# nsp5488/go_raytracer

Hardware: AMD Instinct MI355X
Metric: Msamples/sec (pixels×spp/s) + wall-clock, Cornell Box 800×800×1024spp (higher is better)
Workload: dtype f32

## Files before the change

### go_raytracer_amd/__init__.py

```python
import ctypes as C
import weakref

import numpy as np

from . import _lib
from ._lib import (RT_FT_ALL, RT_FT_BOX, RT_NOISE_MARBLE, RT_NOISE_PERLIN,
                   RT_NOISE_TURBULENT, RtAccumInfo, RtAov, RtCamera, RtDenoiseOpts,
                   RtDenoiseVarOpts, RtCameraDerived, RtError, RtRenderOpts, RtSceneInfo, RtStats, RtTreeView,
                   check, lib)

__all__ = ["Tree", "Camera", "Scene", "Accumulator", "quantize", "format_ppm", "device_count", "RtError",
           "tune", "untune", "tuning", "tune_knobs", "tune_from_env",
           "demo_scene", "DEMO_SCENES", "LoadObjOptions", "DefaultLoadOptions", "quantize_device",
           "format_ppm_device", "denoise", "denoise_device", "denoise_var", "denoise_var_device",
           "RtDenoiseVarOpts"]

DEMO_SCENES = ("book1", "book2", "book3", "simple_light", "quads", "cornell", "cornell_smoke",
               "model")


def _d3(v):
    return _lib.D3(*[float(x) for x in v])


# ... 377 lines not shown
        check(lib().rt_scene_export_qbvh(self._p, None, C.byref(ni), None, C.byref(nn), C.byref(root)))
        items = np.zeros((max(ni.value, 0), 16), np.uint32)
        nodes = np.zeros((max(nn.value, 0), 32), np.uint32)
        check(lib().rt_scene_export_qbvh(self._p, items.ctypes.data or None, C.byref(ni),
                                         nodes.ctypes.data or None, C.byref(nn), C.byref(root)))
        return items, nodes, int(root.value)

    def export_records(self, fill=True):
        ns, sn, nb, counts = C.c_int32(), C.c_int32(), C.c_int32(), (C.c_int32 * 7)()
        check(lib().rt_scene_export_records(self._p, None, C.byref(ns), counts, C.byref(sn), C.byref(nb)))
        pairs = np.zeros((4 * ns.value + sn.value, 4), np.uint32)
        if fill:
            check(lib().rt_scene_export_records(self._p, pairs.ctypes.data or None, C.byref(ns), counts,
                                                C.byref(sn), C.byref(nb)))
        return pairs, ns.value, tuple(counts), sn.value, nb.value

    MODES = {"auto": 0, "wavefront": 1, "fused": 2}

    @staticmethod
    def _opts(seed, device, rank, nranks, path_slots, chunk, profile, stream, mode="auto"):
        o = RtRenderOpts()
        o.mode = Scene.MODES[mode]
        o.seed = seed
        o.device = device
        o.rank = rank
        o.nranks = nranks
        o.path_slots = path_slots
        o.chunk = chunk
        o.flags = _lib.RT_FLAG_PROFILE if profile else 0
        o.stream = stream
# ... 411 lines not shown
```

### go_raytracer_amd/_lib.py

```python
import ctypes as C
import os

_HERE = os.path.dirname(os.path.abspath(__file__))
LIB_PATH = os.environ.get("RT_AMD_LIB") or os.path.join(_HERE, "librt_amd.so")

RT_OK = 0
RT_ERR_INVALID = -1
RT_ERR_UNSUPPORTED = -2
RT_ERR_DEVICE = -3
RT_ERR_OOM = -4
RT_ERR_IO = -5

RT_TEX_SOLID, RT_TEX_CHECKER, RT_TEX_IMAGE, RT_TEX_NOISE = range(4)
RT_NOISE_PERLIN, RT_NOISE_MARBLE, RT_NOISE_TURBULENT = 1, 2, 3
(RT_MAT_LAMBERTIAN, RT_MAT_METAL, RT_MAT_DIELECTRIC, RT_MAT_DIFFUSE_LIGHT,
 RT_MAT_ISOTROPIC) = range(5)
(RT_NODE_LIST, RT_NODE_BVH, RT_NODE_SPHERE, RT_NODE_QUAD, RT_NODE_TRIANGLE,
 RT_NODE_TRANSLATE, RT_NODE_ROTATE_Y, RT_NODE_MEDIUM) = range(8)
RT_FLAG_PROFILE = 1
RT_FLAG_GATHER_RCCL = 2
RT_FT_SPHERE, RT_FT_TRI, RT_FT_METAL, RT_FT_DIEL = 1, 2, 4, 8
RT_FT_MEDIA, RT_FT_CHECKER, RT_FT_IMAGE, RT_FT_NOISE = 16, 32, 64, 128
RT_FT_BOX = 256
RT_FT_ALL = 511
# ... 167 lines not shown
                                C.POINTER(RtObjInfo)]),
    "rt_tree_get_view": (_I, [_P, C.POINTER(RtTreeView)]),
    "rt_camera_derive": (_I, [C.POINTER(RtCamera), C.POINTER(RtCameraDerived)]),
    "rt_scene_create": (_I, [_P, _I, _I, C.POINTER(_P)]),
    "rt_scene_destroy": (_I, [_P]),
    "rt_scene_info_get": (_I, [_P, C.POINTER(RtSceneInfo)]),
    "rt_scene_export_bvh": (_I, [_P, C.c_void_p, C.POINTER(C.c_int32), C.c_void_p,
                                 C.POINTER(C.c_int32), C.POINTER(C.c_uint32)]),
    "rt_scene_export_bvh8": (_I, [_P, C.c_void_p, C.POINTER(C.c_int32), C.c_void_p,
                                  C.POINTER(C.c_int32)]),
    "rt_scene_export_qbvh": (_I, [_P, C.c_void_p, C.POINTER(C.c_int32), C.c_void_p,
                                  C.POINTER(C.c_int32), C.POINTER(C.c_uint32)]),
    "rt_scene_export_records": (_I, [_P, C.c_void_p, C.POINTER(C.c_int32), C.POINTER(C.c_int32),
                                     C.POINTER(C.c_int32), C.POINTER(C.c_int32)]),
    "rt_scene_export_prim_bounds": (_I, [_P, C.c_void_p, C.POINTER(C.c_int32)]),
    "rt_render": (_I, [_P, C.POINTER(RtCamera), C.POINTER(RtRenderOpts), C.c_void_p,
                       C.POINTER(RtStats)]),
    "rt_render_device": (_I, [_P, C.POINTER(RtCamera), C.POINTER(RtRenderOpts), C.c_void_p,
                              C.POINTER(RtStats)]),
    "rt_render_multi": (_I, [_P, C.POINTER(RtCamera), C.POINTER(RtRenderOpts),
                             C.POINTER(C.c_int32), C.c_int32, C.c_void_p, C.POINTER(RtStats)]),
    "rt_render_multi_device": (_I, [_P, C.POINTER(RtCamera), C.POINTER(RtRenderOpts),
                                    C.POINTER(C.c_int32), C.c_int32, C.c_void_p,
                                    C.POINTER(RtStats)]),
    "rt_quantize": (_I, [C.c_void_p, C.c_int64, C.c_void_p]),
    "rt_format_ppm": (C.c_int64, [C.c_void_p, _I, _I, C.c_void_p, C.c_int64]),
    "rt_progress": (_I, [_P, C.POINTER(C.c_uint64), C.POINTER(C.c_uint64)]),
    "rt_quantize_device": (_I, [C.c_void_p, C.c_int64, C.c_void_p, _I, C.c_void_p]),
    "rt_format_ppm_device": (C.c_int64, [C.c_void_p, _I, _I, C.c_void_p, C.c_int64, _I,
                                         C.c_void_p]),
# ... 59 lines not shown
```

### go_raytracer_amd/csrc/host_records.cpp

```cpp
#include <math.h>
#include <string.h>

#include <algorithm>

#include "rt_internal.h"

namespace rt {

void build_leaf_records(const HostScene& h, std::vector<F4>& recs) {
  recs.assign(4 * h.refs.size(), F4{0, 0, 0, 0});
  for (size_t i = 0; i < h.refs.size(); ++i) make_record(h, h.refs[i], &recs[4 * i]);
}
void build_light_records(const HostScene& h, std::vector<F4>& recs) {
  recs.assign(8 * std::max<size_t>(h.lights.size(), 1), F4{0, 0, 0, 0});
  for (size_t i = 0; i < h.lights.size(); ++i) {
    const uint32_t ref = h.lights[i].ref;
    if (ref == PRIM_NONE || (ref >> 30) != PRIM_QUAD) continue;
    make_record(h, ref, &recs[8 * i]);
    const F4* q = &h.quad[5 * (size_t)(ref & 0x3FFFFFFFu)];
    recs[8 * i + 2].w = q[1].w;
    recs[8 * i + 4] = q[0];
    recs[8 * i + 5] = q[1];
    recs[8 * i + 6] = q[2];
  }
// ... 323 lines not shown
  std::stable_sort(ord.begin(), ord.end(), [&](size_t a, size_t b) { return R.larger(a, b); });
  std::vector<char> in_box(h.refs.size(), 0);
  const std::vector<BoxRec> boxes = find_boxes(h, ord, in_box);
  const Groups groups = group_records(R, ord, in_box);
  const SlotOrder so = order_slots(groups, boxes, out.counts);
  out.pairs = interleave_pairs(R, so, boxes);
  out.n_slots = so.slots.size();
  out.n_boxes = (int32_t)boxes.size();
  out.shape = brute_shape_of(out.counts);
  const std::vector<F4> tab = shade_table(h);
  out.shade_n = (int32_t)tab.size();
  out.pairs.insert(out.pairs.end(), tab.begin(), tab.end());
  return out;
}

}
```

### go_raytracer_amd/csrc/host_tune.cpp

```cpp
#include <errno.h>
#include <stdlib.h>
#include <string.h>

#include <algorithm>
#include <map>
#include <mutex>
#include <string>

#include "rt_internal.h"

namespace rt {
namespace {

struct Knob {
  const char* name;
  bool bits;
  char kind;
  double lo, hi;
};
constexpr double kBig = 1e30;
constexpr Knob kKnobs[] = {
    {"RT_BOX_LEAVES", true, 'i', 0, 1},
    {"RT_BIG_SPHERE_R", true, 'f', 0, kBig},
    {"RT_BVH_BUILDER", false, 's', 0, 0},
// ... 2 lines not shown
    {"RT_BVH_LEAF", false, 'i', 1, 64},
    {"RT_BVH_CT", false, 'f', 1e-06, 1000000.0},
    {"RT_BVH_CI", false, 'f', 1e-06, 1000000.0},
    {"RT_BVH_TOP", false, 'i', 1, 1073741824},
    {"RT_THREADS", false, 'i', 1, 1024},
    {"RT_FEATURES_ALL", true, 'i', 0, 1},
    {"RT_BRUTE_MAX", true, 'i', 0, 1048576},
    {"RT_BRUTE_AXIS", false, 'i', 0, 1},
    {"RT_BRUTE_VERT", false, 'i', 0, 1},
    {"RT_BRUTE_BOX", true, 'i', 0, 1},
    {"RT_BRUTE_MIXED", false, 'i', 0, 1},
    {"RT_SHADE_LDS", false, 'i', 0, 1},
    {"RT_TREE", true, 'i', -1, 4},
    {"RT_BRUTE_SMEM", false, 'i', -1, 1},
    {"RT_BRUTE_SHAPE", false, 'i', 0, 1},
    {"RT_QBVH", false, 'i', 0, 1},
    {"RT_CHUNK_NEED", false, 'i', 1, 1048576},
    {"RT_TAIL_FRAC", false, 'i', -1, 1024},
    {"RT_TAIL_K", false, 'i', 1, 4096},
    {"RT_CSUM", false, 'i', 0, 1},
    {"RT_CSUM_MAX_MB", false, 'i', 0, 16777216},
    {"RT_CHUNK_ROWS", false, 'i', -1, 1073741824},
    {"RT_SWEEP", false, 's', 0, 0},
    {"RT_STEP_BUDGET", false, 'i', 1, 1073741824},
    {"RT_SHADE_MIN", false, 'i', 1, 64},
    {"RT_GRAB_MIN", false, 'i', 1, 1048576},
    {"RT_SPLIT_MIN", false, 'i', 0, 1048576},
    {"RT_PARTS_LOG2", false, 'i', 0, 6},
    {"RT_GRAN_LOG2", false, 'i', 0, 20},
    {"RT_WAVE_TIMES", false, 's', 0, 0},
// ... 75 lines not shown
  if (!rt::tune_str(name, &v)) return 0;
  if (buf && cap > 0) {
    const size_t n = std::min<size_t>(v.size(), (size_t)cap - 1);
    memcpy(buf, v.data(), n);
    buf[n] = '\0';
  }
  return (int)v.size() + 1;
}

int rt_brute_shape(const int32_t counts[7]) {
  if (!counts) return rt::set_error(RT_ERR_INVALID, "rt_brute_shape: counts is NULL");
  const rt::BruteCounts c = {counts[0], counts[1], {counts[2], counts[3], counts[4]}, counts[5], counts[6]};
  return rt::brute_shape_of(c);
}

int rt_tune_list(int32_t i, const char** name, int32_t* changes_bits) {
  const int32_t n = (int32_t)(sizeof(rt::kKnobs) / sizeof(rt::kKnobs[0]));
  if (i < 0) return n;
  if (i >= n) return rt::set_error(RT_ERR_INVALID, "rt_tune_list: index %d of %d", i, n);
  if (name) *name = rt::kKnobs[i].name;
  if (changes_bits) *changes_bits = rt::kKnobs[i].bits ? 1 : 0;
  return n;
}

}
```

### go_raytracer_amd/csrc/rt_device.h

```cpp
#pragma once
#include <stdint.h>

namespace rt {

struct alignas(16) F4 {
  float x, y, z, w;
};
struct alignas(8) F2 {
  float x, y;
};

enum : uint32_t { PRIM_SPHERE = 0u, PRIM_QUAD = 1u, PRIM_TRI = 2u, PRIM_MEDIUM = 3u };
constexpr uint32_t PRIM_BOX = 3u;
constexpr uint32_t PRIM_NONE = 0xFFFFFFFFu;
inline constexpr uint32_t prim_ref(uint32_t type, uint32_t idx) { return (type << 30) | idx; }

constexpr uint32_t LEAF_BIT = 0x80000000u;
constexpr int MAX_LEAF = 16;
inline constexpr uint32_t leaf_code(uint32_t first, uint32_t count) {
  return LEAF_BIT | (first << 4) | (count - 1u);
}

constexpr uint32_t CHILD_EMPTY = 0xFFFFFFFEu;

// ... 113 lines not shown
inline constexpr BruteCounts brute_shape(int id) {
  return id == 1   ? BruteCounts{0, 0, {1, 1, 0}, 2 | (3 << 2), 1}
         : id == 2 ? BruteCounts{0, 0, {1, 1, 0}, 2 | (3 << 2), 0}
                   : BruteCounts{0, 0, {0, 0, 0}, 0, 0};
}
inline constexpr bool brute_counts_equal(const BruteCounts& a, const BruteCounts& b) {
  return a.ng == b.ng && a.vy == b.vy && a.ax[0] == b.ax[0] && a.ax[1] == b.ax[1] &&
         a.ax[2] == b.ax[2] && a.mx == b.mx && a.box == b.box;
}
inline constexpr int brute_shape_of(const BruteCounts& c) {
  for (int id = 1; id < kBruteShapeCount; ++id)
    if (brute_counts_equal(c, brute_shape(id))) return id;
  return 0;
}

}
```

### go_raytracer_amd/csrc/rt_fused.h

```cpp
#pragma once
#include "rt_path.h"

namespace rt {

RT_D bool stage_nodes(const Params& P, F4* lnodes, int W) {
  const int nl = min(P.sc.n_nodes, 4 * kLdsNodes / W);
  for (int i = threadIdx.x; i < W * nl; i += blockDim.x) lnodes[i] = P.sc.nodes[i];
  const bool recs = P.recs_lds != 0u;
  if (recs) {
    const int n = 4 * P.sc.n_refs + (P.sc.shade_lds >= 0 ? P.sc.shade_n : 0);
    for (int i = threadIdx.x; i < n; i += blockDim.x) lnodes[W * nl + i] = P.sc.leafprims[i];
  }
  __syncthreads();
  return recs;
}

RT_D void record_trace(const Params& P, const Path& s, const Hit& best) {
  if (s.gpix == P.trace_gpix && s.s0 + s.j == P.trace_sample && (int)s.k < P.trace_cap) {
    P.trace[3 * s.k + 0] = {s.o.x, s.o.y, s.o.z, s.time};
    P.trace[3 * s.k + 1] = {s.d.x, s.d.y, s.d.z, (float)s.k};
    P.trace[3 * s.k + 2] = {best.t, best.u, best.v, bitsf(best.ref)};
  }
}

// ... 96 lines not shown
         : ft == 0u                                                   ? kShortStackMin
         : ft == (FT_SPHERE | FT_TRI | FT_METAL | FT_DIEL | FT_CHECKER) ? (tree == 5 ? MESH_QSHORT : MESH_SHORT)
         : ft == (FT_SPHERE | FT_TRI | FT_METAL)                      ? (tree == 5 ? TRI_QSHORT : TRI_SHORT)
         : ft == FT_SET_BOOK2 ? TEX_SHORT
                                                                      : kShortStack;
}
constexpr unsigned fused_static_lds(uint32_t ft, int tree = 4) {
  return (unsigned)(fused_short(ft, tree) * 4 + fused_wlds(ft, tree) * 12 + 24) * 256u +
         ((ft & FT_NOISE) ? 256u * 16u + 768u : 0u);
}
__shared__ unsigned long long g_tstart[4];
#ifdef RT_DRAIN_TIMES
__shared__ unsigned long long g_tdrain[4];
__shared__ unsigned long long g_dinfo[4][3];
#endif
template <bool LDS, uint32_t FT, int TREE, int SHAPE = 0>
__global__ __launch_bounds__(256, fused_waves(FT, TREE)) void k_fused(Params P) {
  static_assert(SHAPE == 0 || (LDS && FT == 0u && TREE == 0), "shapes: the lean LDS record loop only");
  extern __shared__ F4 lnodes[];
  __shared__ uint32_t lstack[(fused_short(FT, TREE) > 0 ? fused_short(FT, TREE) : 1) * 256];
  __shared__ float lw[3 * fused_wlds(FT, TREE) * 256];
  __shared__ unsigned long long lacc[3 * 256];
  for (int ch = 0; ch < 3; ++ch) lacc[ch * 256 + threadIdx.x] = 0ull;
  if constexpr (HAS(FT_NOISE)) stage_perlin(P.sc);
  if constexpr (cam_mode(FT) == 1) stage_camera(P);
  const bool recs_lds = LDS && TREE != 8 && stage_nodes(P, lnodes, TREE == 4 ? 8 : 4);
#ifdef RT_QTOP
  if constexpr (TREE == 5) {
    const uint32_t nq = 4u * (uint32_t)min(RT_QTOP, P.sc.n_nodes);
    for (uint32_t i = threadIdx.x; i < nq; i += blockDim.x) st_lds(&lnodes[i], ld_glb(P.sc.nodes + i));
  }
#endif
  if (!LDS) __syncthreads();
// ... 104 lines not shown
#ifdef RT_WAVE_SEGS
      wave_segs += n_ready;
#endif

      if (ready) {
        PH_CNT(PH_SHADE_LANES, n_ready);
        PH_CNT(PH_SHADE_ROUNDS, 1);
        PH_T(t_media);
        Hit best = tr.best;
        finish_hit<FT>(P, s, best);
        PH_ADD(PH_MEDIA, t_media);
#ifndef RT_WAVE_SEGS
        ++s.segs;
#endif
        PH_T(t_shade);
        if (shade_core<false, FT>(P, slot, s, best, ws, sa) == OUT_NEED_CHUNK) has = false;
        else {
          trav_init<FT>(P.sc, s.o, s.d, s.time, tr);
#ifdef RT_QROOT
          if constexpr (TREE == 5) trav_root_q(ts, s.o, 0.001f, tr);
#endif
        }
        PH_ADD(PH_SHADE, t_shade);
      }
    }
  }
  PH_ADD(PH_LOOP, t_loop);
#ifdef RT_WAVE_SEGS
  const uint32_t segs = wave_segs;
#else
  uint32_t segs = s.segs;
// ... 38 lines not shown
```

### go_raytracer_amd/csrc/rt_internal.h

```cpp
#pragma once
#include <stdint.h>

#include <atomic>
#include <map>
#include <memory>
#include <mutex>
#include <string>
#include <vector>

#include "rt_abi.h"
#include "rt_device.h"

namespace rt {

int set_error(int code, const char* fmt, ...);

bool tune_str(const char* name, std::string* out);
double tune_num(const char* name, double dflt);
int tune_int(const char* name, int dflt);
int32_t tune_count();

struct Tree {
  std::vector<rt_node> nodes;
  std::vector<std::vector<int32_t>> lists;
// ... 99 lines not shown
               size_t* n_items);
void make_record(const HostScene& h, uint32_t ref, F4* r);
void build_leaf_records(const HostScene& h, std::vector<F4>& recs);
void build_light_records(const HostScene& h, std::vector<F4>& recs);
std::vector<DevMaterial> materials_with_uv_flag(const HostScene& h);
bool tiny_scene(const HostScene& h);
struct RecordPack {
  std::vector<F4> pairs;
  size_t n_slots = 0;
  int32_t shade_n = 0;
  int32_t n_boxes = 0;
  BruteCounts counts{};
  int shape = 0;
};
RecordPack pack_records(const HostScene& h);
int build_bvh_device(HostScene& s, const std::vector<F4>& lo, const std::vector<F4>& hi,
                     const std::vector<uint32_t>& prims, int device);
bool bvh_device_available();
constexpr size_t kBoxLeafMinPrims = 256;
uint32_t scene_features(const HostScene& h, bool* noise_table0 = nullptr);
void release_device(Scene* s);
void release_accums(Scene* s);
struct AovView {
  DevScene sc;
  int tree;
};
int aov_view(Scene* s, int device, AovView* out);

}

// ... 7 lines not shown
```

### go_raytracer_amd/csrc/rt_path.h

```cpp
#pragma once
#include "rt_kernels.h"

namespace rt {

constexpr int kLdsNodes = 384;
constexpr int kLdsWMax = 6;
constexpr int kStack = 64;
constexpr int kShortStack = 12;
constexpr int kShortStackMin = 6;
constexpr int kMaxIt = 1 << 16;
constexpr int kXcd = 8;
constexpr int kMaxParts = 64;
constexpr int kPartStride = 64;

enum : uint32_t { F_PEND = 1u, F_PRE = 2u, F_NONFINITE = 4u };
constexpr uint32_t kCountShift = 8;
constexpr uint32_t F_SPLIT = 0x80u;

#ifdef RT_NO_SPLIT_TREES
constexpr bool kSplitTrees = false;
#else
constexpr bool kSplitTrees = true;
#endif
enum { OUT_DEAD = 0, OUT_ALIVE = 1, OUT_NEED_CHUNK = 2 };
// ... 53 lines not shown
  F4* pend;
  F4* pre;
  F4* stack;
  uint32_t* queue[2];
  Counters* ctr;
  unsigned long long* accum;
  unsigned long long* csum;
  double* side;
  float vlim;
  uint32_t* pflags;
  uint32_t* ostack;
  uint32_t stack_cols;
  F4* trace;
  uint32_t trace_gpix, trace_sample;
  int trace_cap;
};

RT_D uint32_t pack_path(uint32_t j, uint32_t k, uint32_t nst, uint32_t flags) {
  return (j & 0xFFFu) | ((k & 0xFFu) << 12) | ((nst & 0xFFu) << 20) | ((flags & 0xFu) << 28);
}

typedef __attribute__((address_space(3))) uint32_t lds_u32;
typedef __attribute__((address_space(3))) float lds_f32;
typedef __attribute__((address_space(1))) uint32_t glb_u32;
typedef float v4f __attribute__((ext_vector_type(4)));
typedef __attribute__((address_space(3))) v4f lds_v4;
typedef __attribute__((address_space(1))) v4f glb_v4;
typedef float v2f __attribute__((ext_vector_type(2)));
RT_D F4 ld_cst(const F4* p) {
  typedef __attribute__((address_space(4))) const v4f cst_v4;
// ... 1324 lines not shown
      const F4* lr = light_recs + 4;
      Q = ld_cst(lr), U = ld_cst(lr + 1), V = ld_cst(lr + 2);
    } else {
      const F4* lr = light_recs + 8 * (size_t)lo + 4;
      Q = lr[0], U = lr[1], V = lr[2];
    }
    return (xyz(Q) + xyz(U) * s0 + xyz(V) * s1) - origin;
  }
  const F4* tr = sc.tri + 3 * (size_t)idx;
  float r1 = s0, r2 = s1 * (1.0f - r1);
  f3 v0 = xyz(tr[0]), v1 = v0 + xyz(tr[1]), v2 = v0 + xyz(tr[2]);
  f3 p = v0 * (1.0f - r1 - r2) + v1 * r1 + v2 * r2;
  return p - origin;
}

RT_D uint32_t local_pixel(const Params& P, uint32_t chunk) {
  uint32_t sub;
  return chunk_pixel(P, chunk, sub);
}
RT_D unsigned long long to_fixed(float v) {
  const float hi = floorf(v);
  const uint32_t lo = (uint32_t)(fminf(v - hi, 0x1.fffffep-1f) * 4294967296.0f);
  return ((unsigned long long)(uint32_t)(int32_t)hi << 32) | lo;
}
RT_D void add_sample_rare(const Params& P, uint32_t lp, float x, float y, float z) {
  const cst_params* kp = kparams();
  const float c[3] = {x, y, z};
  for (int ch = 0; ch < 3; ++ch) {
    const float v = c[ch];
    if (fabsf(v) < kp->vlim) {
// ... 237 lines not shown
RT_D void start_sample(const Params& P, uint32_t slot, Path& s, uint32_t chunk, uint32_t j) {
  Ids id = chunk_ids<ONE>(P, chunk);
  const rt_u32x4 r = rt_rng_draw(P.seed, id.gpix, id.sample0 + j, RT_STREAM_CAMERA);
  camera_ray_r<CAM>(P, id, id.sample0 + j, r, s.o, s.d, s.time);
  s.spare = rt_spare24(r);
  s.chunk = chunk;
  s.gpix = id.gpix;
  s.s0 = id.sample0;
  s.j = j;
  s.k = 0;
  s.nst = 0;
  s.flags = id.count << kCountShift;
  store_ray<SOA>(P, slot, s);
}

template <bool SOA, uint32_t FT>
RT_D int shade_core(const Params& P, uint32_t slot, Path& s, const Hit& h, const WStack& ws,
                    const SampleAcc& sa) {
  const DevScene& sc = P.sc;
  const f3 o = s.o, d = s.d;
  const float time = s.time;
  const uint32_t ref = h.ref;
  f3 lterm = mk3(0, 0, 0);
  bool term = false;
  rt_u32x4 rcam;
  bool have_rcam = false;
  f3 p = mk3(0, 0, 0), n = mk3(0, 0, 0);
  float u = h.u, v = h.v;
  bool ff = true;
  DevMaterial M;
  bool scat = false;
// ... 124 lines not shown
        if (!cannot) {
          float r0 = (1.0f - ior) * rcp(1.0f + ior);
          r0 = r0 * r0;
          const float x = 1.0f - cs, x2 = x * x;
          float refl_p = r0 + (1.0f - r0) * (x2 * x2 * x);
          refl = refl_p > rt_unit_f(r.v[0]);
        }
        ndir = refl ? reflect(ud, n) : refract(ud, n, ri);
        weight = mk3(1, 1, 1);
      } else {
        const bool iso = HAS(FT_MEDIA) && M.kind == RT_MAT_ISOTROPIC;
        PH_T(t_tex);
        f3 att = ltab ? lcol : tex_value<FT>(sc, M.tex, u, v, p);
        PH_ADD(PH_TEX, t_tex);
        PH_T(t_light);
        Onb b;
        if (!iso) b = make_onb_unit(n);
        if (rt_unit_f(r.v[0]) < 0.5f) {
          ndir = lights_random<FT>(sc, p, r);
        } else if (iso) {
          ndir = uniform_sphere(rt_unit_f(r.v[2]), rt_unit_f(r.v[3]));
        } else {
          ndir = onb_transform(b, cosine_direction(rt_unit_f(r.v[2]), rt_unit_f(r.v[3])));
        }
        float bsdf_pdf, spdf;
        if (iso) {
          bsdf_pdf = 1.0f / (4.0f * kPi);
          spdf = 1.0f / (4.0f * kPi);
        } else {
          f3 ud = unit(ndir);
          bsdf_pdf = fmaxf(0.0f, dot(ud, b.w) * kInvPi);
          float ct = dot(n, ud);
          spdf = fmaxf(0.0f, ct * kInvPi);
        }
#ifdef ABL_NO_LIGHTPDF
        float pdf = 0.5f * 0.01f + 0.5f * bsdf_pdf;
#else
        float pdf = 0.5f * lights_pdf<FT>(sc, p, ndir) + 0.5f * bsdf_pdf;
#endif
        PH_ADD(PH_LIGHT, t_light);
        weight = (att * spdf) * rcp(fmaxf(pdf, sc.pdf_floor));
        clamp_vertex = true;
      }
      if (clamp_vertex) {
        if (s.flags & F_PEND) {
          const f3 pv = get_pend<SOA>(P, slot, s);
#ifndef RT_NO_WEIGHT_MERGE
          const bool merge = kparams()->sc.merge_ok && s.nst > 0 && pv.x >= 0.0f && pv.y >= 0.0f &&
                             pv.z >= 0.0f && pv.x <= 1.0f && pv.y <= 1.0f && pv.z <= 1.0f;
#else
          const bool merge = false;
#endif
          if (merge) {
            f3 top = ws.mul(P, slot, s.nst - 1, pv);
            if (HAS(FT_MEDIA))
              while (s.nst >= 2 && top.x >= 0.0f && top.y >= 0.0f && top.z >= 0.0f &&
                     top.x <= 1.0f && top.y <= 1.0f && top.z <= 1.0f) {
                top = ws.mul(P, slot, s.nst - 2, top);
                --s.nst;
              }
          } else {
            ws.put(P, slot, s.nst, {pv.x, pv.y, pv.z, 0.0f});
            ++s.nst;
// ... 175 lines not shown
```

### go_raytracer_amd/csrc/rt_render.hip

```cpp
#include <hip/hip_runtime.h>
#include <math.h>
#include <stddef.h>
#include <stdio.h>
#include <stdlib.h>
#include <string.h>

#include <algorithm>
#include <chrono>
#include <string>
#include <thread>
#include <vector>

#include <rccl/rccl.h>

#include "rt_hip_util.h"
#include "rt_path.h"
#include "rt_fused.h"
#include "rt_resolve.h"

namespace rt {

RT_D uint32_t queue_slot(const Params& P, const uint32_t* q, const uint32_t* cnt, uint32_t i) {
  uint32_t x = 0;
  while (x + 1 < (uint32_t)kXcd && i >= cnt[x]) {
// ... 118 lines not shown
    }
    out[3 * (size_t)lp + ch] = v;
  }
}

struct DeviceScene {
  int device = -1;
  std::vector<void*> allocs;
  DevScene d{};
  const F4* nodes2 = nullptr;
  const F4* brute_pairs = nullptr;
  size_t brute_slots = 0;
  int32_t shade_n = 0;
  int32_t brute_boxes = 0;
  int brute_shape = 0;
  uint32_t root2 = PRIM_NONE;
  int32_t n_nodes2 = 0;
  const F4* qnodes = nullptr;
  size_t qitems = 0;
  std::mutex qmu;
  bool q_done = false;
  ~DeviceScene() {
    for (void* p : allocs) (void)hipFree(p);
  }
};

struct RenderState {
  int device = -1;
  uint32_t P = 0;
  int depth_cap = 0;
// ... 200 lines not shown
    UP(br, big_recs);
    d.n_big = (int32_t)h.big_refs.size();
  }
  UP(h.lights, lights);
  UP(mats, mats);
  UP(h.texs, texs);
  UP(h.texels, texels);
  UP(h.images, images);
  UP(h.perlins, perlins);
#undef UP
  d.root = h.root4;
  d.n_nodes = (int32_t)(h.nodes4.size() / 8);
  d.n_media = (int32_t)h.media.size();
  d.medium_draws = h.medium_draws;
  d.n_lights = (int32_t)h.lights.size();
  d.pdf_floor = h.lights.empty() ? 0.0f : 1e-30f;
  for (const auto& e : h.lights)
    if (e.ref == PRIM_NONE) d.pdf_floor = 0.0f;
  d.n_refs = (int32_t)h.refs.size();
  d.n_perlins = (int32_t)h.perlins.size();
  d.shade_lds = -1;
  d.shade_n = 0;
  d.merge_ok = 1;
  for (const auto& t : h.texs)
    if (t.kind == RT_TEX_SOLID && !(t.color.x >= 0.0f && t.color.y >= 0.0f && t.color.z >= 0.0f))
      d.merge_ok = 0;
  for (const auto& m : mats)
    if (m.kind == RT_MAT_METAL && !(m.albedo.x >= 0.0f && m.albedo.y >= 0.0f && m.albedo.z >= 0.0f))
      d.merge_ok = 0;
  return RT_OK;
}

template <typename T>
static int dalloc(RenderState* st, T** p, size_t count) {
  void* q = nullptr;
  HIP_OK(hipMalloc(&q, std::max<size_t>(count, 1) * sizeof(T)));
  st->allocs.push_back(q);
  *p = (T*)q;
  return RT_OK;
}

static int ensure_state(SlotState* slot, int device, uint32_t P, int depth_cap, uint32_t npix,
                        bool soa) {
  RenderState* st = slot->st;
// ... 91 lines not shown
RT_FUSED_ILP_KERNELS(RT_FUSED_EXTERN)
#undef RT_FUSED_EXTERN

template <bool LDS>
static const void* fused_for(uint32_t set) {
  switch (set) {
    case kFtSets[0]: return (const void*)k_fused<LDS, kFtSets[0], 4>;
    case kFtSets[1]: return (const void*)k_fused<LDS, kFtSets[1], 4>;
    case kFtSets[2]: return (const void*)k_fused<LDS, kFtSets[2], 4>;
    case kFtSets[3]: return (const void*)k_fused<LDS, kFtSets[3], 4>;
    case kFtSets[4]: return (const void*)k_fused<LDS, kFtSets[4], 4>;
    default: return (const void*)k_fused<LDS, FT_ALL, 4>;
  }
}
static uint32_t pick_set(uint32_t feats) { return pick_ft_set(feats); }
static const void* pick_fused(bool lds, uint32_t set, int tree, int shape = 0) {
  static_assert(kBruteShapeCount == 3, "pick_fused: one kernel per listed shape");
  if (tree == 0 && lds && set == kFtSets[0] && shape == 1) return (const void*)k_fused<true, kFtSets[0], 0, 1>;
  if (tree == 0 && lds && set == kFtSets[0] && shape == 2) return (const void*)k_fused<true, kFtSets[0], 0, 2>;
  if (tree == 0 && lds && set == kFtSets[0]) return (const void*)k_fused<true, kFtSets[0], 0>;
  if (tree == 0 && lds && set == kFtSets[1]) return (const void*)k_fused<true, kFtSets[1], 0>;
  if (tree == 0 && !lds && set == kFtSets[0]) return (const void*)k_fused<false, kFtSets[0], 0>;
  if (tree == 0 && !lds && set == kFtSets[1]) return (const void*)k_fused<false, kFtSets[1], 0>;
  if (tree == 2 && lds && set == kFtSets[0]) return (const void*)k_fused<true, kFtSets[0], 2>;
  if (tree == 2 && lds && set == kFtSets[1]) return (const void*)k_fused<true, kFtSets[1], 2>;
  if (tree == 8) {
#ifdef RT_BVH8_KERNELS
    if (!lds && set == kFtSets[2]) return (const void*)k_fused<false, kFtSets[2], 8>;
    if (!lds && set == kFtSets[3]) return (const void*)k_fused<false, kFtSets[3], 8>;
    if (!lds && set == kFtSets[4]) return (const void*)k_fused<false, kFtSets[4], 8>;
#endif
    return nullptr;
// ... 57 lines not shown
  if (small_set && n_refs > 0 && n_refs <= brute_max) tree = 0;
  else if (small_set && n_refs <= 64 && fits2) tree = 2;
  if (small_set && (env_tree == 4 || (env_tree == 2 && fits2))) tree = env_tree;
  return tree;
}
static bool wants_qbvh(uint32_t ft_set) {
  return env_int("RT_QBVH", 1) != 0 && pick_fused(false, ft_set, 5) != nullptr;
}

struct StructurePlan {
  int tree;
  bool f_lds;
  bool f_recs;
  bool shade_tab;
  int shape;
  const void* kernel;
  size_t lds_bytes;
  bool wants_qbvh;
};
static int plan_structure(const Scene* s, const DeviceScene* ds, uint32_t ft_set, int mode,
                          StructurePlan* out) {
  const size_t n_refs = s->h.refs.size();
  auto slots_for = [&](int tr) { return fused_lds_slots(ft_set, tr); };
  const int env_tree = env_int("RT_TREE", -1);
  int tree = mode == RT_MODE_FUSED ? fused_base_tree(s, ft_set) : 4;
  if (tree == 0 && !ds->brute_pairs) tree = 4;
  if (tree == 2 && !ds->nodes2) tree = 4;
  const size_t lds_slots = slots_for(tree);
  const size_t brute_slots = ds->brute_slots;
  const int smem_env = env_int("RT_BRUTE_SMEM", -1);
// ... 2 lines not shown
  const bool w4 = tree == 4;
  const size_t n_nodes = tree == 4 ? s->h.nodes4.size() / 8 : tree == 2 ? s->h.nodes.size() / 4 : 0;
  const size_t node_slots = w4 ? 2 : 1;
  const bool f_lds = node_slots * n_nodes <= lds_slots && !brute_smem;
  bool shade_tab = tree == 0 && ft_set == 0u && ds->shade_n > 0;
  if (shade_tab && f_lds && brute_slots + (size_t)(ds->shade_n + 3) / 4 > lds_slots) shade_tab = false;
  const size_t rec_slots = tree == 0 ? brute_slots + (shade_tab ? (size_t)(ds->shade_n + 3) / 4 : 0) : n_refs;
  const bool f_recs = f_lds && node_slots * n_nodes + rec_slots <= lds_slots;
  if (tree == 0 && f_lds && !f_recs)
    return set_error(RT_ERR_UNSUPPORTED, "internal: record loop in LDS without its records");
  const bool through_l2 = mode == RT_MODE_FUSED && tree == 4 && !f_lds;
  out->wants_qbvh = through_l2 && wants_qbvh(ft_set);
  if (through_l2 && !s->h.nodes8.empty() && env_tree != 4 && pick_fused(false, ft_set, 8)) tree = 8;
  const int brute_shape_id = tree == 0 && f_lds && ft_set == kFtSets[0] && env_int("RT_BRUTE_SHAPE", 1) != 0
                                 ? ds->brute_shape : 0;
  const void* fused_kernel = pick_fused(f_lds, ft_set, tree, brute_shape_id);
  if (!fused_kernel) return set_error(RT_ERR_UNSUPPORTED, "internal: no fused kernel for this scene");
  const size_t fused_lds = f_lds ? 64 * (node_slots * n_nodes + (f_recs ? rec_slots : 0)) : 0;
  out->tree = tree;
  out->f_lds = f_lds;
  out->f_recs = f_recs;
  out->shade_tab = shade_tab;
  out->shape = brute_shape_id;
  out->kernel = fused_kernel;
  out->lds_bytes = fused_lds;
  return RT_OK;
}
static int take_qbvh(Scene* s, DeviceScene* ds, uint32_t ft_set, StructurePlan* sp) {
  const int rc = ensure_qbvh(s, ds);
  if (rc || !ds->qnodes) return rc;
  sp->tree = 5;
  sp->kernel = pick_fused(false, ft_set, 5);
#ifdef RT_QTOP
  sp->lds_bytes = 64 * std::min<size_t>(RT_QTOP, ds->qitems);
#endif
  return RT_OK;
}

// ... 354 lines not shown
  }
  std::lock_guard<std::mutex> inflight(slot->mu);

  const uint32_t W = (uint32_t)cd.width, H = (uint32_t)cd.height;
  const uint32_t rows = rank_rows(H, o.rank, o.nranks);
  const uint32_t npix = rows * W;
  const uint32_t ss = (uint32_t)cd.spp_sqrt * (uint32_t)cd.spp_sqrt;
  int mode = o.mode;
  if (mode != RT_MODE_WAVEFRONT && mode != RT_MODE_FUSED) mode = RT_MODE_FUSED;
  const int depth_cap = cd.max_depth + 1;
  const uint32_t ft_set = scene_ft_set(s);

  StructurePlan sp;
  if ((rc = plan_structure(s, ds, ft_set, mode, &sp))) return rc;
  if (sp.tree == 4 && sp.wants_qbvh && (rc = take_qbvh(s, ds, ft_set, &sp))) return rc;
  uint32_t P = 0;
  int fused_blocks = 0;
  if (mode == RT_MODE_FUSED) {
    if ((rc = occupancy_blocks(sp.kernel, o.device, &fused_blocks, sp.lds_bytes))) return rc;
    if (o.path_slots > 0) fused_blocks = std::max(1, std::min(fused_blocks, (o.path_slots + 255) / 256));
    P = (uint32_t)fused_blocks * 256u;
  }
  ChunkPlan cp;
  if ((rc = plan_chunks(npix, rows, W, ss, P, o.chunk, ft_set, sp.tree, sp.f_lds, mode, &cp))) return rc;
  const uint32_t n_chunks = cp.n_chunks;
  if (mode != RT_MODE_FUSED) {
    P = o.path_slots > 0 ? (uint32_t)o.path_slots : (1u << 20);
    P = std::max<uint32_t>(256u, std::min<uint32_t>(P, std::max<uint32_t>(n_chunks, 256u)));
    P = (P + 255u) & ~255u;
  }
// ... 12 lines not shown

  hipStream_t stream = (hipStream_t)o.stream;
  if (!stream) {
    if (!st->own_stream) HIP_OK(hipStreamCreateWithFlags(&st->own_stream, hipStreamNonBlocking));
    stream = st->own_stream;
  }

  Params p{};
  p.sc = scene_for_tree(ds, sp.tree);
  if (sp.tree == 0 && sp.shade_tab && sp.f_recs) {
    p.sc.shade_lds = (int32_t)(4 * ds->brute_slots);
    p.sc.shade_n = ds->shade_n;
  }
  set_camera_params(p, cd, o, npix);
  if (!(p.bg[0] >= 0.0f && p.bg[1] >= 0.0f && p.bg[2] >= 0.0f)) p.sc.merge_ok = 0;
  p.K = cp.K;
  p.K2 = cp.K2;
  p.S1 = cp.S1;
  p.n1 = npix * cp.cpp1;
  p.n_chunks = n_chunks;
  p.P = P;
  p.fd_gpix = cp.fd_gpix;
  p.fd_gchunks = cp.fd_gchunks;
  p.fd_gchunks2 = cp.fd_gchunks2;
#ifdef RT_SWEEP_ORDER
  p.gflip = p.gbase = 0u;
#endif
  {
    std::string v;
    if (tune_str("RT_SWEEP", &v) && v == "reverse") {
// ... 336 lines not shown
int rt_progress(const rt_scene* sc, uint64_t* done, uint64_t* total) {
  if (!sc || !done || !total) return rt::set_error(RT_ERR_INVALID, "rt_progress: null");
  rt::Progress& p = const_cast<rt_scene*>(sc)->s.prog;
  std::lock_guard<std::mutex> lk(p.mu);
  *total = p.total;
  *done = p.done;
  if (!p.busy || p.events.empty()) return RT_OK;
  if (hipSetDevice(p.device) != hipSuccess) return rt::set_error(RT_ERR_DEVICE, "rt_progress");
  for (size_t i = 0; i < p.events.size(); ++i) {
    if (hipEventQuery((hipEvent_t)p.events[i]) != hipSuccess) break;
    *done = p.cum[i];
  }
  return RT_OK;
}

int rt_device_count(void) {
  int n = 0;
  if (hipGetDeviceCount(&n) != hipSuccess) return 0;
  return n;
}

}
```

### include/rt_abi.h

```cpp
#ifndef RT_ABI_H
#define RT_ABI_H

#include <stddef.h>
#include <stdint.h>

#ifdef __cplusplus
extern "C" {
#endif

#define RT_ABI_VERSION 4

enum {
  RT_OK = 0,
  RT_ERR_INVALID = -1,
  RT_ERR_UNSUPPORTED = -2,
  RT_ERR_DEVICE = -3,
  RT_ERR_OOM = -4,
  RT_ERR_IO = -5
};

const char* rt_last_error(void);
int rt_abi_version(void);

int rt_tune_set(const char* name, const char* value);
// ... 206 lines not shown
  RT_FT_SPHERE = 1, RT_FT_TRI = 2, RT_FT_METAL = 4, RT_FT_DIEL = 8, RT_FT_MEDIA = 16,
  RT_FT_CHECKER = 32, RT_FT_IMAGE = 64, RT_FT_NOISE = 128,
  RT_FT_BOX = 256
};
int rt_scene_info_get(const rt_scene* s, rt_scene_info* out);

int rt_scene_export_bvh(const rt_scene* s, float* nodes, int32_t* n_nodes, uint32_t* prim_refs,
                        int32_t* n_refs, uint32_t* root);
int rt_scene_export_bvh8(const rt_scene* s, float* nodes, int32_t* n_nodes, uint32_t* refs8,
                         int32_t* n_refs8);
int rt_scene_export_prim_bounds(const rt_scene* s, float* bounds, int32_t* n);
int rt_scene_export_qbvh(const rt_scene* s, float* items, int32_t* n_items, float* nodes4,
                         int32_t* n_nodes4, uint32_t* root4);
int rt_scene_export_records(const rt_scene* s, float* pairs, int32_t* n_slots, int32_t counts[7],
                            int32_t* shade_n, int32_t* n_boxes);

enum {
  RT_FLAG_PROFILE = 1,
  RT_FLAG_GATHER_RCCL = 2
};

enum { RT_MODE_AUTO = 0, RT_MODE_WAVEFRONT = 1, RT_MODE_FUSED = 2 };

typedef struct {
  uint64_t seed;
  int32_t device;
  int32_t rank;
  int32_t nranks;
  int32_t path_slots;
  int32_t chunk;
// ... 132 lines not shown
```

Measured before the change: 24470.

## Specialize fused kernel for a single axis-aligned quad light

Adds a templated LIGHT variant of the fused kernel for scenes whose only light is one axis-aligned quad with unit weight. Light sampling and the light PDF use a constant light block passed in Params with a closed-form single-axis plane intersection, replacing the generic lights_random/lights_pdf loops. The merge_ok and pdf_floor checks become compile-time constants. The cost is more kernel instantiations, a larger Params struct, and extra host-side eligibility checks.

```diff
diff --git a/go_raytracer_amd/__init__.py b/go_raytracer_amd/__init__.py
--- a/go_raytracer_amd/__init__.py
+++ b/go_raytracer_amd/__init__.py
@@ -415,6 +415,18 @@
             check(lib().rt_scene_export_records(self._p, pairs.ctypes.data or None, C.byref(ns), counts,
                                                 C.byref(sn), C.byref(nb)))
         return pairs, ns.value, tuple(counts), sn.value, nb.value
+
+    def lean_light(self):
+        k, n = C.c_int32(), C.c_int32()
+        check(lib().rt_scene_lean_light(self._p, C.byref(k), None, C.byref(n)))
+        block = np.zeros(n.value, np.uint32)
+        check(lib().rt_scene_lean_light(self._p, C.byref(k), block.ctypes.data or None, C.byref(n)))
+        return k.value, block
+
+    def plan_light(self, device=0):
+        k = C.c_int32()
+        check(lib().rt_scene_plan_light(self._p, device, C.byref(k)))
+        return k.value
 
     MODES = {"auto": 0, "wavefront": 1, "fused": 2}
 
diff --git a/go_raytracer_amd/_lib.py b/go_raytracer_amd/_lib.py
--- a/go_raytracer_amd/_lib.py
+++ b/go_raytracer_amd/_lib.py
@@ -205,6 +205,8 @@
     "rt_scene_export_records": (_I, [_P, C.c_void_p, C.POINTER(C.c_int32), C.POINTER(C.c_int32),
                                      C.POINTER(C.c_int32), C.POINTER(C.c_int32)]),
     "rt_scene_export_prim_bounds": (_I, [_P, C.c_void_p, C.POINTER(C.c_int32)]),
+    "rt_scene_lean_light": (_I, [_P, C.POINTER(C.c_int32), C.c_void_p, C.POINTER(C.c_int32)]),
+    "rt_scene_plan_light": (_I, [_P, _I, C.POINTER(C.c_int32)]),
     "rt_render": (_I, [_P, C.POINTER(RtCamera), C.POINTER(RtRenderOpts), C.c_void_p,
                        C.POINTER(RtStats)]),
     "rt_render_device": (_I, [_P, C.POINTER(RtCamera), C.POINTER(RtRenderOpts), C.c_void_p,
diff --git a/go_raytracer_amd/csrc/host_records.cpp b/go_raytracer_amd/csrc/host_records.cpp
--- a/go_raytracer_amd/csrc/host_records.cpp
+++ b/go_raytracer_amd/csrc/host_records.cpp
@@ -361,4 +361,48 @@
   return out;
 }
 
-}
+int32_t scene_merge_ok(const HostScene& h) {
+  for (const auto& t : h.texs)
+    if (t.kind == RT_TEX_SOLID && !(t.color.x >= 0.0f && t.color.y >= 0.0f && t.color.z >= 0.0f))
+      return 0;
+  for (const auto& m : h.mats)
+    if (m.kind == RT_MAT_METAL && !(m.albedo.x >= 0.0f && m.albedo.y >= 0.0f && m.albedo.z >= 0.0f))
+      return 0;
+  return 1;
+}
+float scene_pdf_floor(const HostScene& h) {
+  if (h.lights.empty()) return 0.0f;
+  for (const auto& e : h.lights)
+    if (e.ref == PRIM_NONE) return 0.0f;
+  return 1e-30f;
+}
+
+int lean_light_of(const HostScene& h, LeanLight* block) {
+  if (block) *block = LeanLight{};
+  if (pick_ft_set(h.features) != 0u || h.lights.size() != 1) return 0;
+  const DevLight& e = h.lights[0];
+  if (e.ref == PRIM_NONE || (e.ref >> 30) != PRIM_QUAD || e.weight != 1.0f) return 0;
+  if (scene_merge_ok(h) != 1 || scene_pdf_floor(h) != 1e-30f) return 0;
+  std::vector<F4> lr;
+  build_light_records(h, lr);
+  const float n[3] = {lr[1].x, lr[1].y, lr[1].z}, Q[3] = {lr[0].x, lr[0].y, lr[0].z},
+              A[3] = {lr[2].x, lr[2].y, lr[2].z}, B[3] = {lr[3].x, lr[3].y, lr[3].z};
+  for (int kind = 1; kind < kLeanLightCount; ++kind) {
+    const int a = lean_light_axis(kind);
+    if (a < 0) continue;
+    const int b = (a + 1) % 3, c = (a + 2) % 3;
+    if (!((n[a] == 1.0f || n[a] == -1.0f) && n[b] == 0.0f && n[c] == 0.0f && A[a] == 0.0f &&
+          B[a] == 0.0f))
+      continue;
+    if (block) {
+      const float f[kLeanLightFloats] = {
+          Q[0],    Q[1],    Q[2],    n[a] * lr[1].w, A[0],    A[1],    A[2],    lr[2].w, B[0],    B[1],
+          B[2],    0.0f,    lr[5].x, lr[5].y,        lr[5].z, 0.0f,    lr[6].x, lr[6].y, lr[6].z, 0.0f};
+      memcpy(block->f, f, sizeof f);
+    }
+    return kind;
+  }
+  return 0;
+}
+
+}
diff --git a/go_raytracer_amd/csrc/host_tune.cpp b/go_raytracer_amd/csrc/host_tune.cpp
--- a/go_raytracer_amd/csrc/host_tune.cpp
+++ b/go_raytracer_amd/csrc/host_tune.cpp
@@ -40,6 +40,7 @@
     {"RT_TREE", true, 'i', -1, 4},
     {"RT_BRUTE_SMEM", false, 'i', -1, 1},
     {"RT_BRUTE_SHAPE", false, 'i', 0, 1},
+    {"RT_LEAN_LIGHT", false, 'i', 0, 1},
     {"RT_QBVH", false, 'i', 0, 1},
     {"RT_CHUNK_NEED", false, 'i', 1, 1048576},
     {"RT_TAIL_FRAC", false, 'i', -1, 1024},
@@ -145,6 +146,16 @@
   return rt::brute_shape_of(c);
 }
 
+int rt_scene_lean_light(const rt_scene* sc, int32_t* kind, float* block, int32_t* n_floats) {
+  if (!sc) return rt::set_error(RT_ERR_INVALID, "rt_scene_lean_light: null");
+  rt::LeanLight b;
+  const int k = rt::lean_light_of(sc->s.h, &b);
+  if (kind) *kind = k;
+  if (n_floats) *n_floats = rt::kLeanLightFloats;
+  if (block) memcpy(block, b.f, sizeof b.f);
+  return RT_OK;
+}
+
 int rt_tune_list(int32_t i, const char** name, int32_t* changes_bits) {
   const int32_t n = (int32_t)(sizeof(rt::kKnobs) / sizeof(rt::kKnobs[0]));
   if (i < 0) return n;
diff --git a/go_raytracer_amd/csrc/rt_device.h b/go_raytracer_amd/csrc/rt_device.h
--- a/go_raytracer_amd/csrc/rt_device.h
+++ b/go_raytracer_amd/csrc/rt_device.h
@@ -151,4 +151,11 @@
   return 0;
 }
 
+constexpr int kLeanLightCount = 2;
+inline constexpr int lean_light_axis(int kind) { return kind == 1 ? 1 : -1; }
+constexpr int kLeanLightFloats = 20;
+struct alignas(16) LeanLight {
+  float f[kLeanLightFloats];
+};
+
 }
diff --git a/go_raytracer_amd/csrc/rt_fused.h b/go_raytracer_amd/csrc/rt_fused.h
--- a/go_raytracer_amd/csrc/rt_fused.h
+++ b/go_raytracer_amd/csrc/rt_fused.h
@@ -134,9 +134,11 @@
 __shared__ unsigned long long g_tdrain[4];
 __shared__ unsigned long long g_dinfo[4][3];
 #endif
-template <bool LDS, uint32_t FT, int TREE, int SHAPE = 0>
+template <bool LDS, uint32_t FT, int TREE, int SHAPE = 0, int LIGHT = 0>
 __global__ __launch_bounds__(256, fused_waves(FT, TREE)) void k_fused(Params P) {
   static_assert(SHAPE == 0 || (LDS && FT == 0u && TREE == 0), "shapes: the lean LDS record loop only");
+  static_assert(LIGHT == 0 || (LDS && FT == 0u && TREE == 0), "light kinds: the lean LDS record loop only");
+  static_assert(LIGHT >= 0 && LIGHT < kLeanLightCount, "light kinds: unlisted kind");
   extern __shared__ F4 lnodes[];
   __shared__ uint32_t lstack[(fused_short(FT, TREE) > 0 ? fused_short(FT, TREE) : 1) * 256];
   __shared__ float lw[3 * fused_wlds(FT, TREE) * 256];
@@ -271,7 +273,7 @@
         ++s.segs;
 #endif
         PH_T(t_shade);
-        if (shade_core<false, FT>(P, slot, s, best, ws, sa) == OUT_NEED_CHUNK) has = false;
+        if (shade_core<false, FT, LIGHT>(P, slot, s, best, ws, sa) == OUT_NEED_CHUNK) has = false;
         else {
           trav_init<FT>(P.sc, s.o, s.d, s.time, tr);
 #ifdef RT_QROOT
diff --git a/go_raytracer_amd/csrc/rt_internal.h b/go_raytracer_amd/csrc/rt_internal.h
--- a/go_raytracer_amd/csrc/rt_internal.h
+++ b/go_raytracer_amd/csrc/rt_internal.h
@@ -137,6 +137,9 @@
   int shape = 0;
 };
 RecordPack pack_records(const HostScene& h);
+int32_t scene_merge_ok(const HostScene& h);
+float scene_pdf_floor(const HostScene& h);
+int lean_light_of(const HostScene& h, LeanLight* block);
 int build_bvh_device(HostScene& s, const std::vector<F4>& lo, const std::vector<F4>& hi,
                      const std::vector<uint32_t>& prims, int device);
 bool bvh_device_available();
diff --git a/go_raytracer_amd/csrc/rt_path.h b/go_raytracer_amd/csrc/rt_path.h
--- a/go_raytracer_amd/csrc/rt_path.h
+++ b/go_raytracer_amd/csrc/rt_path.h
@@ -91,6 +91,7 @@
   F4* trace;
   uint32_t trace_gpix, trace_sample;
   int trace_cap;
+  LeanLight ll;
 };
 
 RT_D uint32_t pack_path(uint32_t j, uint32_t k, uint32_t nst, uint32_t flags) {
@@ -1445,6 +1446,33 @@
   return p - origin;
 }
 
+struct LeanLightRegs {
+  F4 q, a, b;
+};
+RT_D LeanLightRegs lean_light_load() {
+  const F4* lb = (const F4*)&kparams()->ll;
+  return {ld_cst(lb), ld_cst(lb + 1), ld_cst(lb + 2)};
+}
+RT_D f3 lean_light_random(const LeanLightRegs& L, f3 origin, const rt_u32x4& r) {
+  const float s0 = rt_unit_f(r.v[2]), s1 = rt_unit_f(r.v[3]);
+  const F4* lb = (const F4*)&kparams()->ll;
+  const F4 U = ld_cst(lb + 3), V = ld_cst(lb + 4);
+  return (xyz(L.q) + xyz(U) * s0 + xyz(V) * s1) - origin;
+}
+template <int KIND>
+RT_D float lean_light_pdf(const LeanLightRegs& L, f3 o, f3 d) {
+  constexpr int A = lean_light_axis(KIND);
+  static_assert(A >= 0 && A < 3, "lean light: a kind with an axis");
+  const float da = comp<A>(d);
+  const float ia = bitsf(pick_by(fbits(rcp(da)), 0x7FC00000u, neg_mask(fabsf(da) - 1e-8f)));
+  const float t = (L.q.w - comp<A>(o)) * ia;
+  const f3 pp = (o + d * t) - xyz(L.q);
+  const float alpha = dot(pp, xyz(L.a)), beta = dot(pp, xyz(L.b));
+  const uint32_t miss = rec_reject_t(t, 0.001f, kInf, alpha, beta);
+  const float dd = dot(d, d);
+  return bitsf(and_not(fbits((t * t * dd) * fsqrt(dd) * rcp(fabsf(da) * L.a.w)), miss));
+}
+
 RT_D uint32_t local_pixel(const Params& P, uint32_t chunk) {
   uint32_t sub;
   return chunk_pixel(P, chunk, sub);
@@ -1712,7 +1740,7 @@
   store_ray<SOA>(P, slot, s);
 }
 
-template <bool SOA, uint32_t FT>
+template <bool SOA, uint32_t FT, int LIGHT = 0>
 RT_D int shade_core(const Params& P, uint32_t slot, Path& s, const Hit& h, const WStack& ws,
                     const SampleAcc& sa) {
   const DevScene& sc = P.sc;
@@ -1867,10 +1895,13 @@
         f3 att = ltab ? lcol : tex_value<FT>(sc, M.tex, u, v, p);
         PH_ADD(PH_TEX, t_tex);
         PH_T(t_light);
+        LeanLightRegs lean;
+        if constexpr (LIGHT != 0) lean = lean_light_load();
         Onb b;
         if (!iso) b = make_onb_unit(n);
         if (rt_unit_f(r.v[0]) < 0.5f) {
-          ndir = lights_random<FT>(sc, p, r);
+          if constexpr (LIGHT != 0) ndir = lean_light_random(lean, p, r);
+          else ndir = lights_random<FT>(sc, p, r);
         } else if (iso) {
           ndir = uniform_sphere(rt_unit_f(r.v[2]), rt_unit_f(r.v[3]));
         } else {
@@ -1889,17 +1920,20 @@
 #ifdef ABL_NO_LIGHTPDF
         float pdf = 0.5f * 0.01f + 0.5f * bsdf_pdf;
 #else
-        float pdf = 0.5f * lights_pdf<FT>(sc, p, ndir) + 0.5f * bsdf_pdf;
+        float lpdf;
+        if constexpr (LIGHT != 0) lpdf = lean_light_pdf<LIGHT>(lean, p, ndir);
+        else lpdf = lights_pdf<FT>(sc, p, ndir);
+        float pdf = 0.5f * lpdf + 0.5f * bsdf_pdf;
 #endif
         PH_ADD(PH_LIGHT, t_light);
-        weight = (att * spdf) * rcp(fmaxf(pdf, sc.pdf_floor));
+        weight = (att * spdf) * rcp(fmaxf(pdf, LIGHT != 0 ? 1e-30f : sc.pdf_floor));
         clamp_vertex = true;
       }
       if (clamp_vertex) {
         if (s.flags & F_PEND) {
           const f3 pv = get_pend<SOA>(P, slot, s);
 #ifndef RT_NO_WEIGHT_MERGE
-          const bool merge = kparams()->sc.merge_ok && s.nst > 0 && pv.x >= 0.0f && pv.y >= 0.0f &&
+          const bool merge = (LIGHT != 0 || kparams()->sc.merge_ok) && s.nst > 0 && pv.x >= 0.0f && pv.y >= 0.0f &&
                              pv.z >= 0.0f && pv.x <= 1.0f && pv.y <= 1.0f && pv.z <= 1.0f;
 #else
           const bool merge = false;
diff --git a/go_raytracer_amd/csrc/rt_render.hip b/go_raytracer_amd/csrc/rt_render.hip
--- a/go_raytracer_amd/csrc/rt_render.hip
+++ b/go_raytracer_amd/csrc/rt_render.hip
@@ -156,6 +156,8 @@
   int32_t shade_n = 0;
   int32_t brute_boxes = 0;
   int brute_shape = 0;
+  int lean_light = 0;
+  LeanLight light_block{};
   uint32_t root2 = PRIM_NONE;
   int32_t n_nodes2 = 0;
   const F4* qnodes = nullptr;
@@ -386,20 +388,13 @@
   d.n_media = (int32_t)h.media.size();
   d.medium_draws = h.medium_draws;
   d.n_lights = (int32_t)h.lights.size();
-  d.pdf_floor = h.lights.empty() ? 0.0f : 1e-30f;
-  for (const auto& e : h.lights)
-    if (e.ref == PRIM_NONE) d.pdf_floor = 0.0f;
+  d.pdf_floor = scene_pdf_floor(h);
   d.n_refs = (int32_t)h.refs.size();
   d.n_perlins = (int32_t)h.perlins.size();
   d.shade_lds = -1;
   d.shade_n = 0;
-  d.merge_ok = 1;
-  for (const auto& t : h.texs)
-    if (t.kind == RT_TEX_SOLID && !(t.color.x >= 0.0f && t.color.y >= 0.0f && t.color.z >= 0.0f))
-      d.merge_ok = 0;
-  for (const auto& m : mats)
-    if (m.kind == RT_MAT_METAL && !(m.albedo.x >= 0.0f && m.albedo.y >= 0.0f && m.albedo.z >= 0.0f))
-      d.merge_ok = 0;
+  d.merge_ok = scene_merge_ok(h);
+  ds->lean_light = lean_light_of(h, &ds->light_block);
   return RT_OK;
 }
 
@@ -521,8 +516,15 @@
   }
 }
 static uint32_t pick_set(uint32_t feats) { return pick_ft_set(feats); }
-static const void* pick_fused(bool lds, uint32_t set, int tree, int shape = 0) {
+static const void* pick_fused(bool lds, uint32_t set, int tree, int shape = 0, int light = 0) {
   static_assert(kBruteShapeCount == 3, "pick_fused: one kernel per listed shape");
+  static_assert(kLeanLightCount == 2, "pick_fused: one kernel per listed shape and light kind");
+  if (light != 0) {
+    if (!(tree == 0 && lds && set == kFtSets[0] && light == 1)) return nullptr;
+    if (shape == 1) return (const void*)k_fused<true, kFtSets[0], 0, 1, 1>;
+    if (shape == 2) return (const void*)k_fused<true, kFtSets[0], 0, 2, 1>;
+    return nullptr;
+  }
   if (tree == 0 && lds && set == kFtSets[0] && shape == 1) return (const void*)k_fused<true, kFtSets[0], 0, 1>;
   if (tree == 0 && lds && set == kFtSets[0] && shape == 2) return (const void*)k_fused<true, kFtSets[0], 0, 2>;
   if (tree == 0 && lds && set == kFtSets[0]) return (const void*)k_fused<true, kFtSets[0], 0>;
@@ -610,6 +612,7 @@
   bool f_recs;
   bool shade_tab;
   int shape;
+  int light;
   const void* kernel;
   size_t lds_bytes;
   bool wants_qbvh;
@@ -642,7 +645,10 @@
   if (through_l2 && !s->h.nodes8.empty() && env_tree != 4 && pick_fused(false, ft_set, 8)) tree = 8;
   const int brute_shape_id = tree == 0 && f_lds && ft_set == kFtSets[0] && env_int("RT_BRUTE_SHAPE", 1) != 0
                                  ? ds->brute_shape : 0;
-  const void* fused_kernel = pick_fused(f_lds, ft_set, tree, brute_shape_id);
+  int light = tree == 0 && f_lds && ft_set == kFtSets[0] && env_int("RT_LEAN_LIGHT", 1) != 0
+                  ? ds->lean_light : 0;
+  if (light != 0 && !pick_fused(f_lds, ft_set, tree, brute_shape_id, light)) light = 0;
+  const void* fused_kernel = pick_fused(f_lds, ft_set, tree, brute_shape_id, light);
   if (!fused_kernel) return set_error(RT_ERR_UNSUPPORTED, "internal: no fused kernel for this scene");
   const size_t fused_lds = f_lds ? 64 * (node_slots * n_nodes + (f_recs ? rec_slots : 0)) : 0;
   out->tree = tree;
@@ -650,6 +656,7 @@
   out->f_recs = f_recs;
   out->shade_tab = shade_tab;
   out->shape = brute_shape_id;
+  out->light = light;
   out->kernel = fused_kernel;
   out->lds_bytes = fused_lds;
   return RT_OK;
@@ -1034,6 +1041,11 @@
   StructurePlan sp;
   if ((rc = plan_structure(s, ds, ft_set, mode, &sp))) return rc;
   if (sp.tree == 4 && sp.wants_qbvh && (rc = take_qbvh(s, ds, ft_set, &sp))) return rc;
+  if (sp.light != 0 && !((float)cd.background[0] >= 0.0f && (float)cd.background[1] >= 0.0f &&
+                         (float)cd.background[2] >= 0.0f)) {
+    sp.light = 0;
+    sp.kernel = pick_fused(sp.f_lds, ft_set, sp.tree, sp.shape, 0);
+  }
   uint32_t P = 0;
   int fused_blocks = 0;
   if (mode == RT_MODE_FUSED) {
@@ -1076,6 +1088,10 @@
   }
   set_camera_params(p, cd, o, npix);
   if (!(p.bg[0] >= 0.0f && p.bg[1] >= 0.0f && p.bg[2] >= 0.0f)) p.sc.merge_ok = 0;
+  if (sp.light != 0) {
+    if (!p.sc.merge_ok) return set_error(RT_ERR_UNSUPPORTED, "internal: lean light kernel without merge_ok");
+    p.ll = ds->light_block;
+  }
   p.K = cp.K;
   p.K2 = cp.K2;
   p.S1 = cp.S1;
@@ -1442,6 +1458,20 @@
   return RT_OK;
 }
 
+int rt_scene_plan_light(rt_scene* sc, int device, int32_t* kind) {
+  if (!sc || !kind) return rt::set_error(RT_ERR_INVALID, "rt_scene_plan_light: null");
+  int rc = rt::device_ok("rt_scene_plan_light", device);
+  if (rc) return rc;
+  rt::DeviceGuard dg;
+  if (hipSetDevice(device) != hipSuccess) return rt::set_error(RT_ERR_DEVICE, "rt_scene_plan_light");
+  rt::DeviceScene* ds = nullptr;
+  if ((rc = rt::ensure_scene(&sc->s, device, &ds))) return rc;
+  rt::StructurePlan sp;
+  if ((rc = rt::plan_structure(&sc->s, ds, rt::scene_ft_set(&sc->s), RT_MODE_FUSED, &sp))) return rc;
+  *kind = sp.light;
+  return RT_OK;
+}
+
 int rt_device_count(void) {
   int n = 0;
   if (hipGetDeviceCount(&n) != hipSuccess) return 0;
diff --git a/include/rt_abi.h b/include/rt_abi.h
--- a/include/rt_abi.h
+++ b/include/rt_abi.h
@@ -244,6 +244,8 @@
                          int32_t* n_nodes4, uint32_t* root4);
 int rt_scene_export_records(const rt_scene* s, float* pairs, int32_t* n_slots, int32_t counts[7],
                             int32_t* shade_n, int32_t* n_boxes);
+int rt_scene_lean_light(const rt_scene* s, int32_t* kind, float* block, int32_t* n_floats);
+int rt_scene_plan_light(rt_scene* s, int device, int32_t* kind);
 
 enum {
   RT_FLAG_PROFILE = 1,
```

Result: faster. 25580, median of 6 (+4.5%).
